# broadinstitute/colab-repeat-finder

Hardware: AMD Instinct MI355X
Metric: Gbp/s scanned (motif 1-50) (higher is better)
Workload: dtype u32 bit planes (2-bit bases)

## Files before the change

colab-repeat-finder_amd/csrc/plan.cpp:

```cpp
#include <algorithm>
#include <cstdio>
#include <cstdlib>
#include <cstring>
#include <string>
#include <vector>

#include "prf_plan.h"

using namespace prf_layout;
static constexpr int MAX_WAVES = PRF_VMAX_WAVES;

bool prf_vertical_plan(u32 kmin, u32 kmax, u32 min_repeats, u32 min_span, prf_vplan *plan) {
    if (kmin < 1 || kmax < kmin || kmax > PRF_VMAX_K || min_repeats < 2) return false;
    struct Item {
        prf_vtask t;
        u32 cost;
    };
    std::vector<Item> items;
    u32 reach = 0;
    u32 covered_to = 0;
    const bool derive_k1 = prf_plan_derives_k1(kmin, kmax, min_repeats, min_span);
    for (u32 k = kmin; k <= kmax; k++) {
        const long long M = prf_plan_min_matches(k, min_repeats, min_span);
        if (M < SMALL_M) {
            Item it;
            it.t.k0 = (unsigned short)k;
            it.t.kind = (unsigned char)M;
            it.t.valid = 1;
            it.t.stride = 1;
            it.t.pad = 0;
            it.cost = M <= 8 ? 660u : (M <= 10 ? 520u : 400u);
            if (derive_k1 && k == 1) {
                it.t.pad = PRF_TASK_DERIVED;
                it.cost = 0;
            }
            if (derive_k1 && k == 2) it.t.pad = PRF_TASK_RAISES_K1;
            items.push_back(it);
            reach = std::max<u32>(reach, 4 * (((u32)T + (u32)M - 1 + k + 3) / 4) - 1);
        } else if (k >= covered_to) {
            const u32 k0 = k & ~3u;
            u32 valid = 0;
            long long mmin[2] = {1ll << 40, 1ll << 40};
            for (u32 kk = 0; kk < 8; kk++) {
                const u32 kx = k0 + kk;
                const long long Mx = prf_plan_min_matches(kx, min_repeats, min_span);
                if (kx >= kmin && kx <= kmax && Mx >= SMALL_M) {
                    valid |= 1u << kk;
                    mmin[kk >> 2] = std::min(mmin[kk >> 2], Mx);
                }
            }
            auto stride_of = [](long long m) { return m >= 39 ? 4u : (m >= 23 ? 2u : 1u); };
            const bool both = (valid & 0x0Fu) && (valid & 0xF0u);
            if (both && stride_of(mmin[0]) != stride_of(mmin[1])) valid &= 0x0Fu;
            const bool half = (valid & 0xF0u) == 0;
            const u32 stride = stride_of(half ? mmin[0] : std::min(mmin[0], mmin[1]));
            Item it;
            it.t.k0 = (unsigned short)k0;
            it.t.kind = 0;
            it.t.valid = (unsigned char)valid;
            it.t.stride = (unsigned char)stride;
            it.t.pad = 0;
            const u32 n_sizes = (u32)__builtin_popcount(valid);
            it.cost = stride == 1 ? 155u + 125u * n_sizes : (stride == 2 ? 105u + 90u * n_sizes : 140u + 40u * n_sizes);
            items.push_back(it);
            reach = std::max<u32>(reach, 24 + k0 + (half ? 11 : 15));
            covered_to = k0 + (half ? 4 : 8);
        }
    }
    if (items.size() > PRF_VMAX_TASKS) return false;
    std::vector<Item> sorted;
    for (const Item &it : items)
        if (!(it.t.pad & PRF_TASK_DERIVED)) sorted.push_back(it);
    const u32 nw = std::max<u32>(1, std::min<u32>(PRF_VMAX_WAVES, (u32)sorted.size()));
    std::vector<std::vector<Item>> bins(nw);
    std::vector<u32> load(nw, 0);
    std::stable_sort(sorted.begin(), sorted.end(), [](const Item &a, const Item &b) { return a.cost > b.cost; });
    constexpr u32 TICKET_COST = 30;
    bool ticket_dealt = nw < (u32)PRF_VMAX_WAVES;
    plan->ticket_wave = nw < (u32)PRF_VMAX_WAVES ? nw : 0;
    for (const Item &it : sorted) {
        if (!ticket_dealt && it.cost <= TICKET_COST) {
            plan->ticket_wave = (u32)(std::min_element(load.begin(), load.end()) - load.begin());
            load[plan->ticket_wave] += TICKET_COST;
            ticket_dealt = true;
        }
        const u32 w = (u32)(std::min_element(load.begin(), load.end()) - load.begin());
        bins[w].push_back(it);
        load[w] += it.cost;
    }
    if (!ticket_dealt) {
        plan->ticket_wave = (u32)(std::min_element(load.begin(), load.end()) - load.begin());
        load[plan->ticket_wave] += TICKET_COST;
    }
    for (int round = 0; round < 64; round++) {
        const u32 hi = (u32)(std::max_element(load.begin(), load.end()) - load.begin());
        bool moved = false;
        for (u32 o = 0; o < nw && !moved; o++) {
            if (o == hi) continue;
            for (size_t i = 0; i < bins[hi].size() && !moved; i++) {
                const u32 ci = bins[hi][i].cost;
                if (std::max(load[hi] - ci, load[o] + ci) < load[hi]) {
                    bins[o].push_back(bins[hi][i]);
                    bins[hi].erase(bins[hi].begin() + (long)i);
                    load[hi] -= ci;
                    load[o] += ci;
                    moved = true;
                    break;
                }
                for (size_t j = 0; j < bins[o].size(); j++) {
                    const u32 cj = bins[o][j].cost;
                    if (cj < ci && std::max(load[hi] - ci + cj, load[o] + ci - cj) < load[hi]) {
                        std::swap(bins[hi][i], bins[o][j]);
                        load[hi] = load[hi] - ci + cj;
                        load[o] = load[o] + ci - cj;
                        moved = true;
                        break;
                    }
                }
            }
        }
        if (!moved) break;
    }
    auto rank_of = [](const Item &it) { return it.t.kind != 0 ? 1 : (it.t.stride < 4 ? 0 : 2); };
    for (auto &bin : bins)
        if (derive_k1) std::stable_sort(bin.begin(), bin.end(), [&](const Item &a, const Item &b) {
            if (rank_of(a) != rank_of(b)) return rank_of(a) < rank_of(b);
            return a.t.kind == 0 && a.t.k0 < b.t.k0;
        });
    for (const Item &it : items)
        if (it.t.pad & PRF_TASK_DERIVED)
            for (auto &bin : bins)
                for (size_t i = 0; i < bin.size(); i++)
                    if (bin[i].t.pad & PRF_TASK_RAISES_K1) {
                        bin.insert(bin.begin() + (long)i + 1, it);
                        break;
                    }
    {
#ifdef PRF_DIAG
        static const u32 prio_cfg = getenv("PRF_PRIO") ? (u32)strtoul(getenv("PRF_PRIO"), nullptr, 0) : 0xA02u;
#else
        const u32 prio_cfg = 0xA02u;
#endif
        plan->prio = prio_cfg;
        const u32 busiest = *std::max_element(load.begin(), load.end());
        plan->slack_waves = 0;
        for (u32 w = 0; w < (u32)PRF_VMAX_WAVES; w++)
            if (w >= nw || 10u * load[w] < 9u * busiest) plan->slack_waves |= 1u << w;
    }
    plan->n_waves = nw;
    plan->n_tasks = 0;
    plan->n_group_k = 0;
    plan->n_exact = 0;
    u32 k_exact0 = ~0u, k_exact1 = 0, n_exact_items = 0;
    for (const Item &it : items)
        if (it.t.kind) {
            k_exact0 = std::min<u32>(k_exact0, it.t.k0);
            k_exact1 = std::max<u32>(k_exact1, it.t.k0);
            n_exact_items++;
        }
    if (n_exact_items && k_exact1 - k_exact0 + 1 != n_exact_items) return false;
    plan->k_exact0 = n_exact_items ? k_exact0 : 0;
    for (u32 w = 0; w < nw; w++) {
        plan->wave_begin[w] = plan->n_tasks;
        for (const Item &it : bins[w]) {
            prf_vtask t = it.t;
            t.item0 = 0;
            if (t.kind == 0) {
                t.item0 = (unsigned short)plan->n_group_k;
                plan->n_group_k += (u32)__builtin_popcount((unsigned)t.valid);
            } else {
                plan->n_exact++;
                t.item0 = (unsigned short)(t.k0 - k_exact0);
            }
            plan->tasks[plan->n_tasks++] = t;
        }
    }
    for (u32 w = nw; w <= PRF_VMAX_WAVES; w++) plan->wave_begin[w] = plan->n_tasks;
    const u32 need_nc = 64 + reach / T;
    plan->nc = need_nc <= 72 ? 72 : 80;
    plan->cof_words = (kmax + 1 + 3) & ~3u;
    plan->lds_bytes = (u32)(SMEM_HDR + (size_t)2 * RG * plan->nc * 16 + (size_t)REC_CAP * sizeof(u64) +
                            (size_t)2 * ROW_CAP_LDS * sizeof(u32) + (size_t)SLOW_CAP * 16 + (size_t)FLAG_CAP * 2 +
                            (size_t)plan->n_group_k * sizeof(u32) + (size_t)plan->cof_words * sizeof(u32));
    plan->per_cu = 0;
    return need_nc <= 80;
}


int prf_plan_json(u32 kmin, u32 kmax, u32 min_repeats, u32 min_span, char *buf, u64 buf_len) {
    std::string out;
    prf_vplan plan;
    if (!prf_vertical_plan(kmin, kmax, min_repeats, min_span, &plan)) {
        out = "{\"path\": \"generic\"}";
    } else {
        char tmp[160];
        snprintf(tmp, sizeof tmp, "{\"path\": \"fused\", \"waves\": %u, \"nc\": %u, \"lds_bytes\": %u, \"tasks\": [", plan.n_waves,
                 plan.nc, plan.lds_bytes);
        out = tmp;
        bool first = true;
        for (u32 w = 0; w < plan.n_waves; w++)
            for (u32 ti = plan.wave_begin[w]; ti < plan.wave_begin[w + 1]; ti++) {
                const prf_vtask &t = plan.tasks[ti];
                snprintf(tmp, sizeof tmp, "%s{\"wave\": %u, \"kind\": %u, \"k0\": %u, \"valid\": %u, \"stride\": %u, \"derive\": %u}",
                         first ? "" : ", ", w, (unsigned)t.kind, (unsigned)t.k0, (unsigned)t.valid, (unsigned)t.stride, (unsigned)(t.pad & 3u));
                out += tmp;
                first = false;
            }
        out += "]}";
    }
    if (out.size() + 1 > buf_len) return -1;
    memcpy(buf, out.c_str(), out.size() + 1);
    return (int)out.size();
}
```

colab-repeat-finder_amd/csrc/scan_vertical.hip:

```cpp
#include <algorithm>
#include <cstdio>
#include <cstdlib>
#include <utility>
#include <vector>

#include "prf_host.h"
#include "prf_static_for.h"
#include "scan_vertical.h"
#include "verify_impl.h"

namespace {

#include "vscan_common.h"
#include "vscan_verify.h"
#include "vscan_tasks.h"

__device__ __forceinline__ void set_prio(u32 p) {
#ifdef PRF_NO_PRIO
    return;
#endif
    if (p == 0u) __builtin_amdgcn_s_setprio(0);
    else if (p == 1u) __builtin_amdgcn_s_setprio(1);
    else if (p == 2u) __builtin_amdgcn_s_setprio(2);
    else __builtin_amdgcn_s_setprio(3);
// ... 41 lines not shown
        if (ut < n_extra) {
            const u32 pw = (u32)__builtin_amdgcn_readfirstlane((int)(ut / (u32)(RG * extra)));
            const u32 erg = (ut / (u32)extra) % (u32)RG, el = ut % (u32)extra;
            const u32 i0 = (erg * 64u + el) * 16u, i1 = i0 + (u32)(RG * 64) * 16u;
            if (pw == 0) {
                ev = ld16(ph, i0);
                en = ld16(ph, i1);
            } else {
                ev = ld16(pL, i0);
                en = ld16(pL, i1);
            }
        }
    }
    __device__ __forceinline__ void clear() {
        const prf_u32x4 z = {0, 0, 0, 0};
        ev = en = z;
        entry = 0;
    }
    __device__ __forceinline__ void store(prf_lds_u4 *vimg, int tid) const {
        const u32 sx = (u32)tid;
        if (sx < n_extra) {
            const u32 p = sx / (u32)(RG * extra), erg = (sx / (u32)extra) % (u32)RG, el = sx % (u32)extra;
            vimg[p * RG * NC + erg * (u32)NC + 64u + el] = (ev >> 1) | (en << 31);
        }
    }
};

__device__ __forceinline__ u32 vscan_skip(const prf_vscan_args &g) {
#ifdef PRF_DIAG
    return g.skip;
#else
    (void)g;
    return 0u;
#endif
}

template <int NC>
__global__ __launch_bounds__(NTH, 6) void prf_vscan_kernel(prf_vscan_args g) {
    constexpr u32 R1_OFF = (u32)SMEM_HDR, R1_BYTES = (u32)(2 * RG * NC * 16);
    constexpr u32 RECS_OFF = R1_OFF + R1_BYTES, KEYS_OFF = RECS_OFF + (u32)REC_CAP * 8u, SLOW_OFF = KEYS_OFF + 2u * (u32)ROW_CAP_LDS * 4u,
                  HOTW_OFF = SLOW_OFF + (u32)SLOW_CAP * 16u, BITEMS_OFF = HOTW_OFF + (u32)FLAG_CAP * 2u;
    static_assert(SLOW_CAP * 16 >= 256, "the all-N stream masks lie in the deferred candidates' list");
    static_assert(2 * LW * 8 <= (int)R1_BYTES, "the window of the linear planes must fit the image's region");
    static_assert((2 * LW / 2 + 63) / 64 <= 5 * MAX_WAVES, "window pieces per wave");
    static_assert(LEAD_OFF == R1_OFF + 2u * (u32)LW * 8u && LEAD_OFF + 2u * LEAD_CAP * 4u <= R1_OFF + R1_BYTES, "the record waves' stream lists lie in R1 behind the window");
    prf_lds_u4 *vimg = (prf_lds_u4 *)(prf_smem + R1_OFF);
    prf_lds_u64 *recs = (prf_lds_u64 *)(prf_smem + RECS_OFF);
    prf_lds_u32 *keys = (prf_lds_u32 *)(prf_smem + KEYS_OFF);
    prf_lds_u32 *nostart = (prf_lds_u32 *)(prf_smem + SLOW_OFF);
    prf_lds_u32 *hotw = (prf_lds_u32 *)(prf_smem + HOTW_OFF);
    prf_lds_u32 *bitems = (prf_lds_u32 *)(prf_smem + BITEMS_OFF);

    const int tid0 = (int)threadIdx.x;
    const int wave = __builtin_amdgcn_readfirstlane(tid0 >> 6);
    auto entry_of = [&](u32 sl) -> u32 { return g.flat_base != ~0u ? g.flat_base + sl : g.launch_list[sl]; };

    set_prio(g.plan.prio & 3u);
    NextRegs<NC> sr;
    sr.load(g, entry_of(blockIdx.x), tid0, wave, R1_OFF);
    for (u32 v = (u32)tid0; v < 8u * g.plan.n_tasks; v += (u32)NTH) {
        const prf_vtask task = g.plan.tasks[v >> 3];
        const u32 kk = v & 7u;
        if (task.kind == 0 && ((task.valid >> kk) & 1u))
            bitems[(u32)task.item0 + (u32)__builtin_popcount((u32)task.valid & ((1u << kk) - 1u))] = ((u32)task.k0 + kk) | ((u32)task.stride << 16);
    }
    {
        prf_lds_u32 *cof_lds = bitems + g.plan.n_group_k;
        for (int i = tid0; i < (int)g.plan.cof_words; i += NTH) cof_lds[i] = prf_cof_table.v[i];
    }
    if (tid0 == 0) {
        TileCtx *tcw = reinterpret_cast<TileCtx *>(prf_smem);
        tcw->H = g.H; tcw->L = g.L; tcw->X = g.X;
        tcw->E = g.E;
        tcw->slab_cap = g.slab_cap;
        tcw->min_repeats = g.min_repeats;
        tcw->min_span = g.min_span;
        tcw->lin_off = R1_OFF;
        tcw->keys_off = KEYS_OFF;
        tcw->slow_off = SLOW_OFF;
        tcw->k_exact0 = g.plan.k_exact0;
        tcw->cof_off = BITEMS_OFF + 4u * g.plan.n_group_k;
    }

    const u32 xcd = blockIdx.x & 7u;
    const u32 first_ticket = (gridDim.x - xcd + 7u) >> 3;
    u64 *ticket_word = g.counters + (PRF_CNT_SHARD0 + xcd * PRF_CNT_SHARD_STRIDE + PRF_SH_TILE_TICKET);
    prf_lds_u32 *next_words = (prf_lds_u32 *)(prf_smem + HDR_NEXT);
    u32 slot_next = 0;
    u32 parity = 0;
    prf_lds_u32 *wg_stats = (prf_lds_u32 *)(prf_smem + HDR_STATS);
    if (tid0 == 0) wg_stats[0] = wg_stats[1] = 0;
    for (u32 slot = blockIdx.x; slot < g.n_launch; slot = slot_next, parity ^= 1u) {
    int wave_s = wave;
    asm volatile("" : "+s"(wave_s));
    u32 ones = ~0u;
    asm volatile("" : "+s"(ones));
    int tid = wave_s * 64 + (int)__builtin_amdgcn_mbcnt_hi(ones, __builtin_amdgcn_mbcnt_lo(ones, 0u));
    asm volatile("" : "+v"(tid));
    const int lane = tid & 63;
    const u32 entry = sr.entry;
    const bool hasx = (entry & PRF_LAUNCH_MIXED) != 0;
    const u64 tile = entry & ~PRF_LAUNCH_MIXED;
    prf_lds_u32 *cnt = smem_cnt(parity);

    PRF_STAMP(0);
#ifdef PRF_STAMPS
    if (g.dbg && lane == 0) g.dbg[((u64)slot * MAX_WAVES + wave) * PRF_STAMP_SLOTS + 12] = __builtin_amdgcn_s_memrealtime();
#endif
    set_prio(g.plan.prio & 3u);
    {
        sr.store(vimg, tid);
        if (hasx && tid < 64) {
            const u32 *px = reinterpret_cast<const u32 *>(g.X + tile * PRF_TILE_WORDS);
            u32 m = 0;
#pragma unroll 1
            for (u32 b0 = 0; b0 < 32u; b0 += 8u) {
                u32 v[8];
                static_for<0, 8>([&](auto bc) { v[decltype(bc)::value] = *(prf_glb_cu32 *)(px + ((b0 + (u32)decltype(bc)::value) * 64u + (u32)tid)); });
                static_for<0, 8>([&](auto bc) { m |= (v[decltype(bc)::value] == ~0u ? 1u : 0u) << (b0 + (u32)decltype(bc)::value); });
            }
            nostart[tid] = m;
        }
        if (tid < (int)CNT_N) cnt[tid] = 0;
        if (tid == 0) {
            TileCtx *tcw = reinterpret_cast<TileCtx *>(prf_smem);
            tcw->w0 = tile * PRF_TILE_WORDS - LIN_PRE;
            tcw->xz_lo = hasx ? 0 : tile * PRF_TILE;
            tcw->xz_hi = hasx ? 0 : (tile + 2) * PRF_TILE;
            tcw->slab = (prf_glb_u64 *)(g.slabs + (u64)slot * g.slab_cap);
            tcw->tile_base = tile * PRF_TILE;
            tcw->has_lin = 0u;
            tcw->cnt_off = (u32)HDR_CNT + 4u * CNT_N * parity;
        }
    }
    PRF_STAMP(1);
    __syncthreads();
    PRF_STAMP(2);

    set_prio(((g.plan.slack_waves >> wave) & 1u) ? (g.plan.prio >> 4) & 3u : (g.plan.prio >> 2) & 3u);
    Emit em;
    em.recs = recs;
    em.cnt = cnt;
    em.lane = lane;
#ifdef PRF_STAMPS
    u64 *task_dbg = g.dbg ? g.dbg + ((u64)slot * MAX_WAVES + wave) * PRF_STAMP_SLOTS : nullptr;
#else
    u64 *task_dbg = nullptr;
#endif
    {
        u32 allow = hasx ? ~nostart[lane] : ~0u;
        if (vscan_skip(g) & 1u) allow = 0u;
        run_tasks<NC>((prf_lds_cu4 *)vimg, hotw, nostart, g.plan, wave, lane, hasx, allow, em, task_dbg);
    }
    constexpr u32 WIN_UNITS = (u32)LW;
    constexpr u32 WIN_PIECES = (WIN_UNITS + 63u) / 64u;
    static_assert(WIN_PIECES == 17, "the window's pieces are dealt 9 + 8 to the first two waves to arrive");
    prf_u32x4 wv[9];
    u32 order = 0;
    {
        if (lane == 0) order = atomicAdd((u32 *)(cnt + CNT_ROWS0), 1u);
        order = (u32)__builtin_amdgcn_readfirstlane((int)order);
        const long long w0 = (long long)(tile * PRF_TILE_WORDS) - LIN_PRE;
        const u64 *wh = g.H + w0, *wl = g.L + w0;
        const prf_u32x4 z = {0, 0, 0, 0};
        static_for<0, 9>([&](auto ic) { wv[decltype(ic)::value] = z; });
        if (order < 2u) {
            const u32 first = order * 9u, n = order ? 8u : 9u;
            static_for<0, 9>([&](auto ic) {
                constexpr u32 i = (u32)decltype(ic)::value;
                if (i < n) {
                    const u32 u = (first + i) * 64u + (u32)lane;
                    const u64 *src = u < (u32)LW / 2u ? wh + 2u * u : wl + 2u * (u - (u32)LW / 2u);
                    if (u < WIN_UNITS) wv[i] = *reinterpret_cast<const prf_u32x4 *>(src);
                }
            });
        }
    }
    u64 ticket = 0;
    const bool ticket_thread = order == 0u && lane == 0;
    if (ticket_thread) ticket = atomicAdd(ticket_word, 1ull);
    PRF_STAMP(3);
    __syncthreads();
    {
        if (order < 2u) {
            const u32 first = order * 9u, n = order ? 8u : 9u;
            static_for<0, 9>([&](auto ic) {
                constexpr u32 i = (u32)decltype(ic)::value;
                if (i < n) {
                    const u32 u = (first + i) * 64u + (u32)lane;
                    if (u < WIN_UNITS) *(prf_lds_u4 *)(prf_smem + R1_OFF + 16u * u) = wv[i];
                }
            });
        }
        const prf_u32x4 n0 = *(prf_lds_cu4 *)(cnt + CNT_ROWS);
        for (u32 i = (u32)tid; i < (u32)ROW_CAP_LDS; i += (u32)NTH) {
            const u32 q = i / (u32)QCAP, j = i - q * (u32)QCAP;
            const u32 n0q = q == 0u ? n0.x : (q == 1u ? n0.y : (q == 2u ? n0.z : n0.w));
            if (j >= n0q) keys[i] = quarter_pad(q);
        }
        if (tid == 0) {
            reinterpret_cast<TileCtx *>(prf_smem)->has_lin = 1u;
            cnt[CNT_ROWS0] = n0.x;
            cnt[CNT_ROWS0 + 1u] = n0.y;
            cnt[CNT_ROWS0 + 2u] = n0.z;
            cnt[CNT_ROWS0 + 3u] = n0.w;
            cnt[CNT_OVF0] = cnt[CNT_OVF];
            cnt[CNT_LONG0] = cnt[CNT_LONG];
        }
    }
    u32 slot_pre = 0, entry_pre = entry;
    if (ticket_thread) {
        slot_pre = (first_ticket + (u32)ticket) * 8u + xcd;
        if (slot_pre < g.n_launch) entry_pre = entry_of(slot_pre);
    }
    __syncthreads();
    PRF_STAMP(4);

    set_prio(wave < MAX_WAVES / 2 ? (g.plan.prio >> 6) & 3u : (g.plan.prio >> 8) & 3u);
    const u32 *xw = hasx ? reinterpret_cast<const u32 *>(g.X + ((long long)(tile * PRF_TILE_WORDS) - LIN_PRE)) : nullptr;
    typedef const unsigned short __attribute__((address_space(3))) prf_lds_cu16;
    u32 n_recs = cnt[CNT_RECS], n_flags = cnt[CNT_FLAGS];
    {
        if (tid == 0) {
            const u32 early = cnt[CNT_EARLY];
            wg_stats[0] += n_flags + n_recs + early;
            wg_stats[1] += early;
        }
        n_recs = n_recs < (u32)REC_CAP ? n_recs : (u32)REC_CAP;
        n_flags = n_flags < (u32)FLAG_CAP ? n_flags : (u32)FLAG_CAP;
#ifdef PRF_STAMPS
        if (g.dbg && tid == 0) g.dbg[((u64)slot * MAX_WAVES + 0) * PRF_STAMP_SLOTS + 11] = (u64)n_flags | ((u64)n_recs << 32);
#endif
        if (vscan_skip(g) & 2u) n_flags = 0;
        if (vscan_skip(g) & 4u) n_recs = 0;
        verify_all((prf_lds_cu64 *)recs, n_recs, (prf_lds_cu32 *)bitems, (vscan_skip(g) & 8u) ? 0u : g.plan.n_group_k, (prf_lds_cu16 *)hotw, n_flags, xw, (u32)tid, task_dbg);
    }
    set_prio((g.plan.prio >> 10) & 3u);
    if (ticket_thread) {
        next_words[0] = slot_pre;
        next_words[1] = entry_pre;
    }
    PRF_STAMP(5);
    __syncthreads();
    {
        const u32 n_slow = (u32)__builtin_amdgcn_readfirstlane((int)cnt[CNT_SLOW]);
        if (n_slow) {
            if (n_slow <= (u32)SLOW_CAP) {
                if ((u32)tid < n_slow) {
                    prf_lds_u64 *slow = (prf_lds_u64 *)(prf_smem + SLOW_OFF);
                    slow_item(slow[2u * (u32)tid], slow[2u * (u32)tid + 1u]);
                }
            } else {
                if (tid == 0) {
                    for (u32 q = 0; q < 4u; q++) cnt[CNT_ROWS + q] = cnt[CNT_ROWS0 + q];
                    cnt[CNT_OVF] = cnt[CNT_OVF0];
                    cnt[CNT_LONG] = cnt[CNT_LONG0];
                }
                __syncthreads();
                verify_general((prf_lds_cu64 *)recs, n_recs, (prf_lds_cu32 *)bitems, g.plan.n_group_k, (prf_lds_cu16 *)hotw, n_flags, (u32)tid);
            }
            __syncthreads();
        }
    }
    PRF_STAMP(6);
    const u64 nw = *(prf_lds_u64 *)next_words;
    slot_next = (u32)__builtin_amdgcn_readfirstlane((int)(u32)nw);
    const u32 entry_next = (u32)(nw >> 32);
    u32 nq0, nq1, nq2, nq3;
    {
        const prf_u32x4 c = *(prf_lds_cu4 *)(cnt + CNT_ROWS);
        const bool none = (vscan_skip(g) & 16u) != 0;
        nq0 = none ? 0u : (u32)__builtin_amdgcn_readfirstlane((int)c.x);
        nq1 = none ? 0u : (u32)__builtin_amdgcn_readfirstlane((int)c.y);
        nq2 = none ? 0u : (u32)__builtin_amdgcn_readfirstlane((int)c.z);
        nq3 = none ? 0u : (u32)__builtin_amdgcn_readfirstlane((int)c.w);
    }
    const u32 n_rows = nq0 + nq1 + nq2 + nq3;
    const bool dense = nq0 > (u32)QCAP || nq1 > (u32)QCAP || nq2 > (u32)QCAP || nq3 > (u32)QCAP;
    const u32 n_long = (u32)__builtin_amdgcn_readfirstlane((int)cnt[CNT_LONG]);
    u64 *slab = g.slabs + (u64)slot * g.slab_cap;
    const u32 n_store = n_rows < g.slab_cap ? n_rows : g.slab_cap;
    bool unsorted = false;
    if (tid == 0) {
        g.slab_count[slot] = n_rows;
        if (n_store && !(vscan_skip(g) & 32u)) atomicAdd(&g.block_sum[slot >> g.gather_shift], n_store);
    }

    if (dense) {
        constexpr u32 R1_ROWS = R1_BYTES / 8u;
        const u32 m0 = nq0 < (u32)QCAP ? nq0 : (u32)QCAP, m1 = nq1 < (u32)QCAP ? nq1 : (u32)QCAP, m2 = nq2 < (u32)QCAP ? nq2 : (u32)QCAP,
                  m3 = nq3 < (u32)QCAP ? nq3 : (u32)QCAP;
        const u32 n_ovf = n_rows - (m0 + m1 + m2 + m3);
        const u32 s1 = nq0, s2 = nq0 + nq1, s3 = s2 + nq2;
        auto pick = [](u32 q, u32 a0, u32 a1, u32 a2, u32 a3) -> u32 { return q == 0u ? a0 : (q == 1u ? a1 : (q == 2u ? a2 : a3)); };
        if (n_rows <= g.slab_cap && n_rows <= R1_ROWS) {
            prf_lds_u32 *k2 = (prf_lds_u32 *)(prf_smem + R1_OFF), *v2 = k2 + R1_ROWS;
            prf_lds_u32 *fill = cnt + CNT_ROWS0;
            if (tid < 4) fill[tid] = pick((u32)tid, m0, m1, m2, m3);
            for (u32 i = (u32)tid; i < (u32)ROW_CAP_LDS; i += (u32)NTH) {
                const u32 q = i / (u32)QCAP, j = i - q * (u32)QCAP;
                if (j < pick(q, m0, m1, m2, m3)) {
                    const u32 at = pick(q, 0u, s1, s2, s3) + j;
                    k2[at] = keys[i];
                    v2[at] = keys[ROW_CAP_LDS + i];
                }
            }
            __syncthreads();
            for (u32 i = (u32)tid; i < n_ovf; i += (u32)NTH) {
                const u64 r = slab[i];
                const u32 q = (u32)r >> 30;
                const u32 at = pick(q, 0u, s1, s2, s3) + atomicAdd((u32 *)(fill + q), 1u);
                k2[at] = (u32)r;
                v2[at] = (u32)(r >> 32);
            }
            for (u32 i = n_rows + (u32)tid; i < ((n_rows + 3u) & ~3u); i += (u32)NTH) k2[i] = 0xFFFFFFFFu;
            __syncthreads();
            typedef __attribute__((address_space(3))) const prf_u32x4 prf_lds_ckey4;
            prf_lds_ckey4 *k4 = (prf_lds_ckey4 *)k2;
            for (u32 r = (u32)tid; r < n_rows; r += (u32)NTH) {
                const u32 mine = k2[r], kv = v2[r];
                const u32 q = mine >> 30;
                const u32 lo = pick(q, 0u, s1, s2, s3), hi = lo + pick(q, nq0, nq1, nq2, nq3);
                const u32 u_lo = lo >> 2, u_hi = (hi + 3u) >> 2;
                u32 rank = 4u * u_lo;
#pragma unroll 4
                for (u32 u = u_lo; u < u_hi; u++) {
                    const prf_u32x4 v = k4[u];
                    rank += (v.x < mine ? 1u : 0u) + (v.y < mine ? 1u : 0u) + (v.z < mine ? 1u : 0u) + (v.w < mine ? 1u : 0u);
                }
                slab[rank] = (u64)mine | ((u64)kv << 32);
            }
            __syncthreads();
        } else {
            for (u32 i = (u32)tid; i < (u32)ROW_CAP_LDS; i += (u32)NTH) {
                const u32 q = i / (u32)QCAP, j = i - q * (u32)QCAP;
                const u32 at = n_ovf + pick(q, 0u, m0, m0 + m1, m0 + m1 + m2) + j;
                if (j < pick(q, m0, m1, m2, m3) && at < g.slab_cap) slab[at] = (u64)keys[i] | ((u64)keys[ROW_CAP_LDS + i] << 32);
            }
            unsorted = true;
        }
    }

    if (slot_next < g.n_launch) sr.load(g, entry_next, tid, wave, R1_OFF);
    else sr.clear();

    PRF_RANK_DECL();
    {
        const u32 nq = wave_s == 0 ? nq0 : (wave_s == 1 ? nq1 : (wave_s == 2 ? nq2 : nq3));
        const u32 below = wave_s == 0 ? 0u : (wave_s == 1 ? nq0 : (wave_s == 2 ? nq0 + nq1 : nq0 + nq1 + nq2));
        if (nq && !dense) {
            const u32 lg = nq > 32u ? 0u : (nq > 16u ? 1u : 2u);
            const u32 P = 1u << lg, part = (u32)lane & (P - 1u);
            const u32 units = (nq + 3u) >> 2;
            prf_lds_u32 *sub = keys + (u32)wave_s * (u32)QCAP;
            typedef __attribute__((address_space(3))) const prf_u32x4 prf_lds_ckey4;
            prf_lds_ckey4 *k4 = (prf_lds_ckey4 *)sub + part;
            for (u32 row0 = 0; row0 < nq; row0 += 64u >> lg) {
                const u32 row = row0 + ((u32)lane >> lg);
                const u32 r = row < nq ? row : 0u;
                PRF_RANK_T0();
                const u32 mine = sub[r];
                const u32 kv = sub[ROW_CAP_LDS + r];
                u32 rank = 0;
                auto batch = [&](u32 u0, auto nc) {
                    constexpr u32 N = (u32)decltype(nc)::value;
                    prf_u32x4 v[N];
                    static_for<0, (int)N>([&](auto jc) { v[decltype(jc)::value] = k4[u0 + (u32)decltype(jc)::value * P]; });
                    if constexpr (N == 4u) asm volatile("" : "+v"(v[0]), "+v"(v[1]), "+v"(v[2]), "+v"(v[3]));
                    else asm volatile("" : "+v"(v[0]), "+v"(v[1]));
                    u32 bits = 0;
                    static_for<0, (int)N>([&](auto jc) {
                        constexpr u32 j = (u32)decltype(jc)::value;
                        bits = __builtin_amdgcn_alignbit(bits, v[j].x - mine, 31);
                        bits = __builtin_amdgcn_alignbit(bits, v[j].y - mine, 31);
                        bits = __builtin_amdgcn_alignbit(bits, v[j].z - mine, 31);
                        bits = __builtin_amdgcn_alignbit(bits, v[j].w - mine, 31);
                    });
                    rank += (u32)__builtin_popcount(bits);
                };
                for (u32 u0 = 0; u0 < units; u0 += 4u * P) {
                    if (units - u0 > 2u * P) batch(u0, std::integral_constant<u32, 4>{});
                    else batch(u0, std::integral_constant<u32, 2>{});
                }
                if (P >= 2u) rank += (u32)__builtin_amdgcn_update_dpp(0, (int)rank, 0xB1, 0xF, 0xF, true);
// ... 72 lines not shown
```

colab-repeat-finder_amd/csrc/vscan_tasks.h:

```cpp

struct Emit {
    prf_lds_u64 *recs;
    prf_lds_u32 *cnt;
    int lane;
#ifdef PRF_STAMPS
    u64 t_push_g = 0, t_push_f = 0;
#endif

    static constexpr u32 DENSE_FLAGS = 4;
    __device__ __forceinline__ void push_flags(u32 word, u32 e, u32 k, prf_lds_u32 *flag_words) {
        typedef __attribute__((address_space(3))) unsigned short prf_lds_u16;
        prf_lds_u16 *list = (prf_lds_u16 *)flag_words;
        const u32 pc = (u32)__builtin_popcount(word);
        if (__builtin_amdgcn_ballot_w64(pc > DENSE_FLAGS) != 0) {
            push_flags_levels(word, e, k, list);
            return;
        }
        if (word == 0) return;
        u32 at = atomicAdd((u32 *)(cnt + CNT_FLAGS), pc);
        const u32 tag = (u32)lane | (e << 11);
        if (at + pc <= (u32)FLAG_CAP) {
            prf_lds_u16 *p = list + at;
            do {
                *p++ = (unsigned short)(tag | ((u32)__builtin_ctz(word) << 6));
// ... 267 lines not shown
                    const u32 win = window_or<M, t>(mm, o3);
                    if constexpr (!ECHO) {
                        if constexpr (t >= 0) hot = bitop3<(TA | (~TB & TC)) & 0xFF>(hot, win, prev);
                        if constexpr (t == 0) {
                            if (relax) hot |= ~win;
                        }
                    } else if constexpr (t >= 0) {
                        if constexpr (t == 0 || t % SEG == 1) seg = ~win & prev;
                        else seg = bitop3<(TA | (~TB & TC)) & 0xFF>(seg, win, prev);
                        if constexpr (t == 0) {
                            if (relax) seg |= ~win;
                        }
                        if constexpr (t % SEG == 0 || t == T - 1) {
                            hot = bitop3<(TA | (TB & TC)) & 0xFF>(hot, seg, prim[(t + SEG - 1) / SEG]);
                            if constexpr (K == 2) hot1 = bitop3<(TA | (TB & ~TC)) & 0xFF>(hot1, seg, prim[(t + SEG - 1) / SEG]);
                        }
                    }
                    prev = win;
                }
            }
        });
    });
    return (u64)hot | ((u64)hot1 << 32);
}

template <int K, int M, int NC>
__device__ __attribute__((noinline)) u32 coarse_stream(prf_lds_cu4 *vimg, int lane, bool relax) {
    constexpr int PS = RG * NC;
    constexpr int G = M >= 11 ? 4 : 2, C = (M + 1) / G - 1;
    constexpr int NJ = T / G + 1;
    constexpr int NGRP = NJ + C;
    constexpr int NR = T + G * C;
    constexpr int NG = (NR + K + 3) / 4;
    static_assert(C >= 2 && 4 * NG <= 2 * T, "a coarse task reads its own lane and the next one");
    int lane_o = lane;
    asm volatile("" : "+v"(lane_o));
    prf_lds_cu4 *lane_base = vimg + lane_o;
    u32 q0[4], q1[4];
    {
        const int pl = (lane + 63) & 63;
        prf_lds_cu4 *pp = vimg + pl + (RG - 1) * NC;
        prf_u32x4 v0 = pp[0], v1 = pp[PS];
        if (lane == 0) {
            v0 <<= 1;
            v1 <<= 1;
        }
        q0[0] = v0.x; q0[1] = v0.y; q0[2] = v0.z; q0[3] = v0.w;
        q1[0] = v1.x; q1[1] = v1.y; q1[2] = v1.z; q1[3] = v1.w;
    }
    u32 r0[4 * NG], r1[4 * NG];
    u32 grp[NGRP];
    u32 hot = 0;
    auto load_slot = [&](auto gc) {
        constexpr int g = decltype(gc)::value;
        if constexpr (g < NG) {
            prf_lds_cu4 *ps = slot_of<NC>(lane_base, g);
            const prf_u32x4 v0 = ps[0], v1 = ps[PS];
            r0[4 * g] = v0.x; r0[4 * g + 1] = v0.y; r0[4 * g + 2] = v0.z; r0[4 * g + 3] = v0.w;
            r1[4 * g] = v1.x; r1[4 * g + 1] = v1.y; r1[4 * g + 2] = v1.z; r1[4 * g + 3] = v1.w;
        }
    };
    auto h = [&](auto rc) -> u32 { constexpr int r = decltype(rc)::value; if constexpr (r < 0) return q0[r + 4]; else return r0[r]; };
    auto l = [&](auto rc) -> u32 { constexpr int r = decltype(rc)::value; if constexpr (r < 0) return q1[r + 4]; else return r1[r]; };
    load_slot(std::integral_constant<int, 0>{});
    static_for<0, NG>([&](auto gc) {
        constexpr int g = decltype(gc)::value;
        load_slot(std::integral_constant<int, g + 1>{});
        __builtin_amdgcn_sched_barrier(0);
        static_for<0, 4>([&](auto jc) {
            constexpr int i = 4 * g + decltype(jc)::value - K;
            if constexpr (i >= -1 && i < NR && (i + 1) % G == 0) {
                constexpr int j = (i + 1) / G - 1, first = G * j;
                u32 t = h(std::integral_constant<int, first>{}) ^ h(std::integral_constant<int, first + K>{});
                t = or_xor(t, l(std::integral_constant<int, first>{}), l(std::integral_constant<int, first + K>{}));
                static_for<1, G>([&](auto ic) {
                    constexpr int r = first + decltype(ic)::value;
                    t = or_xor(t, h(std::integral_constant<int, r>{}), h(std::integral_constant<int, r + K>{}));
                    t = or_xor(t, l(std::integral_constant<int, r>{}), l(std::integral_constant<int, r + K>{}));
                });
                if constexpr (j == -1) {
                    if (lane == 0) t |= 1u;
                }
                grp[j + 1] = t;
                constexpr int w = j - C + 1;
                if constexpr (w >= 0 && w < NJ) {
                    u32 win;
                    if constexpr (C == 2) win = grp[w + 1] | grp[w + 2];
                    else if constexpr (C == 3) win = or3(grp[w + 1], grp[w + 2], grp[w + 3]);
                    else if constexpr (C == 4) win = or3(grp[w + 1], grp[w + 2], grp[w + 3]) | grp[w + 4];
                    else win = or3(or3(grp[w + 1], grp[w + 2], grp[w + 3]), grp[w + 4], grp[w + 5]);
                    static_assert(C <= 5, "window of at most five groups");
                    hot = bitop3<(TA | (~TB & TC)) & 0xFF>(hot, win, grp[w]);
                    if constexpr (w == 0) {
                        if (relax) hot |= ~win;
                    }
                }
            }
        });
    });
    return hot;
}

constexpr int exact_variants() { return (SMALL_M - 1) * SMALL_M / 2; }
constexpr int exact_variant_of(int K, int M) { return (K - 1) * (2 * SMALL_M - K) / 2 + (M - K); }
constexpr int exact_variant_k(int v) {
    int K = 1;
    while (exact_variant_of(K + 1, K + 1) <= v) K++;
    return K;
}
template <int LO, int HI, int NC>
__device__ __forceinline__ u64 exact_dispatch(prf_lds_cu4 *vimg, int lane, bool relax, u32 v) {
    if constexpr (LO == HI) {
        constexpr int K = exact_variant_k(LO), M = K + (LO - exact_variant_of(K, K));
        static_assert(M >= K && M < SMALL_M && exact_variant_of(K, M) == LO, "variant numbering");
        if constexpr (M >= 9) return coarse_stream<K, M, NC>(vimg, lane, relax);
        else return exact_stream<K, M, NC>(vimg, lane, relax);
    } else {
        constexpr int MID = (LO + HI) / 2;
        if (v <= (u32)MID) return exact_dispatch<LO, MID, NC>(vimg, lane, relax, v);
        return exact_dispatch<MID + 1, HI, NC>(vimg, lane, relax, v);
    }
}

template <int NC>
__device__ __forceinline__ u64 exact_any(prf_lds_cu4 *vimg, int lane, bool relax, u32 k, u32 M) {
    const u32 v = (k - 1u) * (2u * (u32)SMALL_M - k) / 2u + (M - k);
    return exact_dispatch<0, exact_variants() - 1, NC>(vimg, lane, relax, v);
}

template <int NC>
__device__ __forceinline__ void run_tasks(prf_lds_cu4 *vimg, prf_lds_u32 *hotw, prf_lds_u32 *k1w, const prf_vplan &plan, int wave, int lane, bool relax,
                                          u32 allow, Emit &em, u64 *dbg) {
    const u32 t_end = plan.wave_begin[wave + 1];
    {
        u32 a = (u32)(__UINTPTR_TYPE__)vimg;
        asm volatile("" : "+s"(a));
        vimg = (prf_lds_cu4 *)(__UINTPTR_TYPE__)a;
    }
#ifdef PRF_STAMPS
    u64 t_call = 0;
#endif
    for (u32 ti = plan.wave_begin[wave]; ti < t_end; ti++) {
        static_assert(sizeof(prf_vtask) == 8 && alignof(prf_vtask) == 4, "a task is read as two dwords");
        const u32 *tw = reinterpret_cast<const u32 *>(&plan.tasks[ti]);
        const u32 tw0 = (u32)__builtin_amdgcn_readfirstlane((int)tw[0]), tw1 = (u32)__builtin_amdgcn_readfirstlane((int)tw[1]);
        prf_vtask task;
        task.k0 = (unsigned short)(tw0 & 0xFFFFu);
        task.kind = (unsigned char)((tw0 >> 16) & 0xFFu);
        task.valid = (unsigned char)(tw0 >> 24);
        task.stride = (unsigned char)(tw1 & 0xFFu);
        task.pad = (unsigned char)((tw1 >> 8) & 0xFFu);
        task.item0 = (unsigned short)(tw1 >> 16);
#ifdef PRF_STAMPS
        if (dbg && lane == 0 && ti - plan.wave_begin[wave] < 8u) dbg[8 + (ti - plan.wave_begin[wave])] = __builtin_amdgcn_s_memtime();
#endif
        if (task.kind == 0) {
            const bool half = (task.valid & 0xF0u) == 0;
            if (task.stride == 1 && !relax) {
                if (half) group_task<NC, true, true>(vimg, lane, task.k0, task.valid, 1u, allow, em);
                else group_task<NC, true, false>(vimg, lane, task.k0, task.valid, 1u, allow, em);
            } else {
                if (half) group_task<NC, false, true>(vimg, lane, task.k0, task.valid, task.stride, allow, em);
                else group_task<NC, false, false>(vimg, lane, task.k0, task.valid, task.stride, allow, em);
            }
        } else {
            u32 word;
#ifdef PRF_STAMPS
            const u64 tc0 = __builtin_amdgcn_s_memtime();
#endif
            if ((task.pad & PRF_TASK_DERIVED) && !relax) {
                word = k1w[lane];
            } else {
                const u64 words = exact_any<NC>(vimg, lane, relax, task.k0, task.kind);
                word = (u32)words & allow;
                if ((task.pad & PRF_TASK_RAISES_K1) && !relax) k1w[lane] = (u32)(words >> 32) & allow;
            }
#ifdef PRF_STAMPS
            asm volatile("" ::"v"(word));
            const u64 tc1 = __builtin_amdgcn_s_memtime();
            t_call += tc1 - tc0;
#endif
            em.push_flags(word, task.item0, task.k0, hotw);
#ifdef PRF_STAMPS
            em.t_push_f += __builtin_amdgcn_s_memtime() - tc1;
#endif
        }
    }
#ifdef PRF_STAMPS
    if (dbg && lane == 0) dbg[15] = (t_call & 0x3FFFFFull) | ((em.t_push_f & 0x1FFFFFull) << 22) | ((em.t_push_g & 0x1FFFFFull) << 43);
#endif
}
```

Baseline: 6665.

## Rebalance wave task deal with measured prices, local search and exhaustive search

Replaces the per-task cost model with new task prices and folds the k=1 derived handover cost into the task that raises it. Greedy dealing is now followed by move/swap local search and, for small task counts, an exhaustive branch-and-bound over wave assignments. The ticket wave is chosen from the final loads, and wave priority is raised after the task phase. The window registers are left uninitialised instead of being zeroed. The plan is cached per parameter set so repeated host calls skip the search. The aim is to shorten the busiest wave's critical path, at the risk that the price model does not match the real kernel.

```diff
diff --git a/colab-repeat-finder_amd/csrc/plan.cpp b/colab-repeat-finder_amd/csrc/plan.cpp
--- a/colab-repeat-finder_amd/csrc/plan.cpp
+++ b/colab-repeat-finder_amd/csrc/plan.cpp
@@ -10,7 +10,77 @@
 using namespace prf_layout;
 static constexpr int MAX_WAVES = PRF_VMAX_WAVES;
 
-bool prf_vertical_plan(u32 kmin, u32 kmax, u32 min_repeats, u32 min_span, prf_vplan *plan) {
+namespace {
+constexpr u32 FIRST_TASK = 300;
+constexpr u32 K1_HANDOVER = 1660;
+
+u32 task_price(const prf_vtask &t) {
+    if (t.kind != 0) {
+        if (t.pad & PRF_TASK_DERIVED) return K1_HANDOVER;
+        const u32 k = t.k0, M = t.kind;
+        if (M <= 8) {
+            if (k == 2 && M == 7) return 4000;
+            if (k == 3 && M == 6) return 4040;
+            if (k == 4 && M == 8) return 3960;
+            return 4000;
+        }
+        return M <= 10 ? 3630 : 3600;
+    }
+    const u32 n = (u32)__builtin_popcount((unsigned)t.valid);
+    if (t.stride == 1) return 3050 + 400 * n;
+    if (t.stride == 2) return 3550 + 200 * n;
+    return 2900 + 100 * n;
+}
+
+#ifdef PRF_DIAG
+const u32 WINDOW_W = getenv("PRF_PLAN_W") ? (u32)strtoul(getenv("PRF_PLAN_W"), nullptr, 0) : 0u;
+#else
+constexpr u32 WINDOW_W = 0;
+#endif
+
+constexpr u32 PRIO_HANDOVER = 3, PRIO_FLAGS = 2;
+
+struct DealKey {
+    u32 obj, a4, a34;
+    bool operator<(const DealKey &o) const { return obj != o.obj ? obj < o.obj : (a4 != o.a4 ? a4 < o.a4 : a34 < o.a34); }
+};
+DealKey deal_key(const u32 (&load)[PRF_VMAX_WAVES]) {
+    u32 a[PRF_VMAX_WAVES];
+    std::copy(load, load + PRF_VMAX_WAVES, a);
+    std::sort(a, a + PRF_VMAX_WAVES);
+    return DealKey{std::max(a[PRF_VMAX_WAVES - 1], a[1] + WINDOW_W), a[PRF_VMAX_WAVES - 1], a[PRF_VMAX_WAVES - 1] + a[PRF_VMAX_WAVES - 2]};
+}
+
+struct DealSearch {
+    const std::vector<u32> &cost;
+    std::vector<u32> where, best_where;
+    u32 load[PRF_VMAX_WAVES] = {};
+    DealKey best;
+    long nodes = 0;
+    static constexpr long MAX_NODES = 400000;
+    void go(size_t i) {
+        if (++nodes > MAX_NODES) return;
+        const DealKey here = deal_key(load);
+        if (!(here < best)) return;
+        if (i == cost.size()) {
+            best = here;
+            best_where = where;
+            return;
+        }
+        for (u32 w = 0; w < (u32)PRF_VMAX_WAVES; w++) {
+            bool seen = false;
+            for (u32 v = 0; v < w; v++) seen = seen || load[v] == load[w];
+            if (seen) continue;
+            load[w] += cost[i];
+            where[i] = w;
+            go(i + 1);
+            load[w] -= cost[i];
+        }
+    }
+};
+}
+
+static bool build_plan(u32 kmin, u32 kmax, u32 min_repeats, u32 min_span, prf_vplan *plan) {
     if (kmin < 1 || kmax < kmin || kmax > PRF_VMAX_K || min_repeats < 2) return false;
     struct Item {
         prf_vtask t;
@@ -29,12 +99,9 @@
             it.t.valid = 1;
             it.t.stride = 1;
             it.t.pad = 0;
-            it.cost = M <= 8 ? 660u : (M <= 10 ? 520u : 400u);
-            if (derive_k1 && k == 1) {
-                it.t.pad = PRF_TASK_DERIVED;
-                it.cost = 0;
-            }
+            if (derive_k1 && k == 1) it.t.pad = PRF_TASK_DERIVED;
             if (derive_k1 && k == 2) it.t.pad = PRF_TASK_RAISES_K1;
+            it.cost = task_price(it.t);
             items.push_back(it);
             reach = std::max<u32>(reach, 4 * (((u32)T + (u32)M - 1 + k + 3) / 4) - 1);
         } else if (k >= covered_to) {
@@ -60,8 +127,7 @@
             it.t.valid = (unsigned char)valid;
             it.t.stride = (unsigned char)stride;
             it.t.pad = 0;
-            const u32 n_sizes = (u32)__builtin_popcount(valid);
-            it.cost = stride == 1 ? 155u + 125u * n_sizes : (stride == 2 ? 105u + 90u * n_sizes : 140u + 40u * n_sizes);
+            it.cost = task_price(it.t);
             items.push_back(it);
             reach = std::max<u32>(reach, 24 + k0 + (half ? 11 : 15));
             covered_to = k0 + (half ? 4 : 8);
@@ -69,58 +135,77 @@
     }
     if (items.size() > PRF_VMAX_TASKS) return false;
     std::vector<Item> sorted;
+    u32 handover = 0;
     for (const Item &it : items)
-        if (!(it.t.pad & PRF_TASK_DERIVED)) sorted.push_back(it);
-    const u32 nw = std::max<u32>(1, std::min<u32>(PRF_VMAX_WAVES, (u32)sorted.size()));
+        if (it.t.pad & PRF_TASK_DERIVED) handover = it.cost;
+        else sorted.push_back(it);
+    for (Item &it : sorted)
+        if (it.t.pad & PRF_TASK_RAISES_K1) it.cost += handover;
+    std::stable_sort(sorted.begin(), sorted.end(), [](const Item &a, const Item &b) { return a.cost > b.cost; });
+    const size_t n_dealt = sorted.size();
+    std::vector<u32> cost(n_dealt), where(n_dealt, 0);
+    u32 load[PRF_VMAX_WAVES] = {};
+    for (size_t i = 0; i < n_dealt; i++) {
+        cost[i] = sorted[i].cost;
+        where[i] = (u32)(std::min_element(load, load + PRF_VMAX_WAVES) - load);
+        load[where[i]] += cost[i];
+    }
+    for (bool better = true; better;) {
+        better = false;
+        DealKey cur = deal_key(load);
+        for (size_t i = 0; i < n_dealt && !better; i++) {
+            for (u32 w = 0; w < (u32)PRF_VMAX_WAVES && !better; w++) {
+                if (w == where[i]) continue;
+                u32 l2[PRF_VMAX_WAVES];
+                std::copy(load, load + PRF_VMAX_WAVES, l2);
+                l2[where[i]] -= cost[i];
+                l2[w] += cost[i];
+                if (deal_key(l2) < cur) {
+                    std::copy(l2, l2 + PRF_VMAX_WAVES, load);
+                    where[i] = w;
+                    better = true;
+                }
+            }
+            for (size_t j = i + 1; j < n_dealt && !better; j++) {
+                if (where[i] == where[j] || cost[i] == cost[j]) continue;
+                u32 l2[PRF_VMAX_WAVES];
+                std::copy(load, load + PRF_VMAX_WAVES, l2);
+                l2[where[i]] = l2[where[i]] - cost[i] + cost[j];
+                l2[where[j]] = l2[where[j]] - cost[j] + cost[i];
+                if (deal_key(l2) < cur) {
+                    std::copy(l2, l2 + PRF_VMAX_WAVES, load);
+                    std::swap(where[i], where[j]);
+                    better = true;
+                }
+            }
+        }
+    }
+    constexpr size_t EXHAUSTIVE_TASKS = 16;
+    if (n_dealt <= EXHAUSTIVE_TASKS) {
+        DealSearch ds{cost, std::vector<u32>(n_dealt, 0), where};
+        ds.best = deal_key(load);
+        ds.go(0);
+        where = ds.best_where;
+    }
+    u32 n_used = 0;
+    {
+        u32 name[PRF_VMAX_WAVES];
+        std::fill(name, name + PRF_VMAX_WAVES, ~0u);
+        for (size_t i = 0; i < n_dealt; i++)
+            if (name[where[i]] == ~0u) name[where[i]] = n_used++;
+        for (size_t i = 0; i < n_dealt; i++) where[i] = name[where[i]];
+    }
+    const u32 nw = std::max<u32>(1, n_used);
     std::vector<std::vector<Item>> bins(nw);
-    std::vector<u32> load(nw, 0);
-    std::stable_sort(sorted.begin(), sorted.end(), [](const Item &a, const Item &b) { return a.cost > b.cost; });
-    constexpr u32 TICKET_COST = 30;
-    bool ticket_dealt = nw < (u32)PRF_VMAX_WAVES;
-    plan->ticket_wave = nw < (u32)PRF_VMAX_WAVES ? nw : 0;
-    for (const Item &it : sorted) {
-        if (!ticket_dealt && it.cost <= TICKET_COST) {
-            plan->ticket_wave = (u32)(std::min_element(load.begin(), load.end()) - load.begin());
-            load[plan->ticket_wave] += TICKET_COST;
-            ticket_dealt = true;
-        }
-        const u32 w = (u32)(std::min_element(load.begin(), load.end()) - load.begin());
-        bins[w].push_back(it);
-        load[w] += it.cost;
-    }
-    if (!ticket_dealt) {
-        plan->ticket_wave = (u32)(std::min_element(load.begin(), load.end()) - load.begin());
-        load[plan->ticket_wave] += TICKET_COST;
-    }
-    for (int round = 0; round < 64; round++) {
-        const u32 hi = (u32)(std::max_element(load.begin(), load.end()) - load.begin());
-        bool moved = false;
-        for (u32 o = 0; o < nw && !moved; o++) {
-            if (o == hi) continue;
-            for (size_t i = 0; i < bins[hi].size() && !moved; i++) {
-                const u32 ci = bins[hi][i].cost;
-                if (std::max(load[hi] - ci, load[o] + ci) < load[hi]) {
-                    bins[o].push_back(bins[hi][i]);
-                    bins[hi].erase(bins[hi].begin() + (long)i);
-                    load[hi] -= ci;
-                    load[o] += ci;
-                    moved = true;
-                    break;
-                }
-                for (size_t j = 0; j < bins[o].size(); j++) {
-                    const u32 cj = bins[o][j].cost;
-                    if (cj < ci && std::max(load[hi] - ci + cj, load[o] + ci - cj) < load[hi]) {
-                        std::swap(bins[hi][i], bins[o][j]);
-                        load[hi] = load[hi] - ci + cj;
-                        load[o] = load[o] + ci - cj;
-                        moved = true;
-                        break;
-                    }
-                }
-            }
-        }
-        if (!moved) break;
-    }
+    std::fill(load, load + PRF_VMAX_WAVES, 0u);
+    for (size_t i = 0; i < n_dealt; i++) {
+        Item it = sorted[i];
+        load[where[i]] += it.cost;
+        if (it.t.pad & PRF_TASK_RAISES_K1) it.cost -= handover;
+        bins[where[i]].push_back(it);
+    }
+    for (u32 w = 0; w < nw; w++) load[w] += FIRST_TASK;
+    plan->ticket_wave = (u32)(std::min_element(load, load + PRF_VMAX_WAVES) - load);
     auto rank_of = [](const Item &it) { return it.t.kind != 0 ? 1 : (it.t.stride < 4 ? 0 : 2); };
     for (auto &bin : bins)
         if (derive_k1) std::stable_sort(bin.begin(), bin.end(), [&](const Item &a, const Item &b) {
@@ -136,13 +221,14 @@
                         break;
                     }
     {
+        constexpr u32 PRIO_DEFAULT = 0x0A02u | (PRIO_HANDOVER << 12) | (PRIO_FLAGS << 6);
 #ifdef PRF_DIAG
-        static const u32 prio_cfg = getenv("PRF_PRIO") ? (u32)strtoul(getenv("PRF_PRIO"), nullptr, 0) : 0xA02u;
+        static const u32 prio_cfg = getenv("PRF_PRIO") ? (u32)strtoul(getenv("PRF_PRIO"), nullptr, 0) : PRIO_DEFAULT;
 #else
-        const u32 prio_cfg = 0xA02u;
+        const u32 prio_cfg = PRIO_DEFAULT;
 #endif
         plan->prio = prio_cfg;
-        const u32 busiest = *std::max_element(load.begin(), load.end());
+        const u32 busiest = *std::max_element(load, load + PRF_VMAX_WAVES);
         plan->slack_waves = 0;
         for (u32 w = 0; w < (u32)PRF_VMAX_WAVES; w++)
             if (w >= nw || 10u * load[w] < 9u * busiest) plan->slack_waves |= 1u << w;
@@ -186,6 +272,23 @@
     return need_nc <= 80;
 }
 
+bool prf_vertical_plan(u32 kmin, u32 kmax, u32 min_repeats, u32 min_span, prf_vplan *plan) {
+    struct Last {
+        u32 key[4];
+        bool have, ok;
+        prf_vplan plan;
+    };
+    thread_local Last last = {};
+    if (!(last.have && last.key[0] == kmin && last.key[1] == kmax && last.key[2] == min_repeats && last.key[3] == min_span)) {
+        last.have = false;
+        last.plan = prf_vplan{};
+        last.ok = build_plan(kmin, kmax, min_repeats, min_span, &last.plan);
+        last.key[0] = kmin; last.key[1] = kmax; last.key[2] = min_repeats; last.key[3] = min_span;
+        last.have = true;
+    }
+    *plan = last.plan;
+    return last.ok;
+}
 
 int prf_plan_json(u32 kmin, u32 kmax, u32 min_repeats, u32 min_span, char *buf, u64 buf_len) {
     std::string out;
@@ -193,16 +296,17 @@
     if (!prf_vertical_plan(kmin, kmax, min_repeats, min_span, &plan)) {
         out = "{\"path\": \"generic\"}";
     } else {
-        char tmp[160];
-        snprintf(tmp, sizeof tmp, "{\"path\": \"fused\", \"waves\": %u, \"nc\": %u, \"lds_bytes\": %u, \"tasks\": [", plan.n_waves,
-                 plan.nc, plan.lds_bytes);
+        char tmp[240];
+        snprintf(tmp, sizeof tmp, "{\"path\": \"fused\", \"waves\": %u, \"nc\": %u, \"lds_bytes\": %u, \"window\": %u, \"first_task\": %u, \"tasks\": [",
+                 plan.n_waves, plan.nc, plan.lds_bytes, (unsigned)WINDOW_W, (unsigned)FIRST_TASK);
         out = tmp;
         bool first = true;
         for (u32 w = 0; w < plan.n_waves; w++)
             for (u32 ti = plan.wave_begin[w]; ti < plan.wave_begin[w + 1]; ti++) {
                 const prf_vtask &t = plan.tasks[ti];
-                snprintf(tmp, sizeof tmp, "%s{\"wave\": %u, \"kind\": %u, \"k0\": %u, \"valid\": %u, \"stride\": %u, \"derive\": %u}",
-                         first ? "" : ", ", w, (unsigned)t.kind, (unsigned)t.k0, (unsigned)t.valid, (unsigned)t.stride, (unsigned)(t.pad & 3u));
+                snprintf(tmp, sizeof tmp, "%s{\"wave\": %u, \"kind\": %u, \"k0\": %u, \"valid\": %u, \"stride\": %u, \"derive\": %u, \"price\": %u}",
+                         first ? "" : ", ", w, (unsigned)t.kind, (unsigned)t.k0, (unsigned)t.valid, (unsigned)t.stride, (unsigned)(t.pad & 3u),
+                         (unsigned)task_price(t));
                 out += tmp;
                 first = false;
             }
diff --git a/colab-repeat-finder_amd/csrc/scan_vertical.hip b/colab-repeat-finder_amd/csrc/scan_vertical.hip
--- a/colab-repeat-finder_amd/csrc/scan_vertical.hip
+++ b/colab-repeat-finder_amd/csrc/scan_vertical.hip
@@ -217,6 +217,8 @@
         if (vscan_skip(g) & 1u) allow = 0u;
         run_tasks<NC>((prf_lds_cu4 *)vimg, hotw, nostart, g.plan, wave, lane, hasx, allow, em, task_dbg);
     }
+    PRF_STAMP(17);
+    set_prio((g.plan.prio >> 12) & 3u);
     constexpr u32 WIN_UNITS = (u32)LW;
     constexpr u32 WIN_PIECES = (WIN_UNITS + 63u) / 64u;
     static_assert(WIN_PIECES == 17, "the window's pieces are dealt 9 + 8 to the first two waves to arrive");
@@ -225,10 +227,12 @@
     {
         if (lane == 0) order = atomicAdd((u32 *)(cnt + CNT_ROWS0), 1u);
         order = (u32)__builtin_amdgcn_readfirstlane((int)order);
+#ifdef PRF_STAMPS
+        if (g.dbg && lane == 0) g.dbg[((u64)slot * MAX_WAVES + wave) * PRF_STAMP_SLOTS + 18] = order;
+#endif
         const long long w0 = (long long)(tile * PRF_TILE_WORDS) - LIN_PRE;
         const u64 *wh = g.H + w0, *wl = g.L + w0;
-        const prf_u32x4 z = {0, 0, 0, 0};
-        static_for<0, 9>([&](auto ic) { wv[decltype(ic)::value] = z; });
+        asm("" : "=v"(wv[0]), "=v"(wv[1]), "=v"(wv[2]), "=v"(wv[3]), "=v"(wv[4]), "=v"(wv[5]), "=v"(wv[6]), "=v"(wv[7]), "=v"(wv[8]));
         if (order < 2u) {
             const u32 first = order * 9u, n = order ? 8u : 9u;
             static_for<0, 9>([&](auto ic) {
@@ -244,8 +248,19 @@
     u64 ticket = 0;
     const bool ticket_thread = order == 0u && lane == 0;
     if (ticket_thread) ticket = atomicAdd(ticket_word, 1ull);
-    PRF_STAMP(3);
+#ifdef PRF_STAMPS
+    {
+        const u64 t3 = __builtin_amdgcn_s_memtime();
+        if (order < 2u) asm volatile("s_waitcnt vmcnt(0)" ::: "memory");
+        const u64 t20 = __builtin_amdgcn_s_memtime();
+        if (g.dbg && lane == 0) {
+            g.dbg[((u64)slot * MAX_WAVES + wave) * PRF_STAMP_SLOTS + 3] = t3;
+            g.dbg[((u64)slot * MAX_WAVES + wave) * PRF_STAMP_SLOTS + 20] = t20;
+        }
+    }
+#endif
     __syncthreads();
+    PRF_STAMP(19);
     {
         if (order < 2u) {
             const u32 first = order * 9u, n = order ? 8u : 9u;
@@ -257,6 +272,7 @@
                 }
             });
         }
+        PRF_STAMP(21);
         const prf_u32x4 n0 = *(prf_lds_cu4 *)(cnt + CNT_ROWS);
         for (u32 i = (u32)tid; i < (u32)ROW_CAP_LDS; i += (u32)NTH) {
             const u32 q = i / (u32)QCAP, j = i - q * (u32)QCAP;
@@ -272,6 +288,7 @@
             cnt[CNT_OVF0] = cnt[CNT_OVF];
             cnt[CNT_LONG0] = cnt[CNT_LONG];
         }
+        PRF_STAMP(22);
     }
     u32 slot_pre = 0, entry_pre = entry;
     if (ticket_thread) {
@@ -294,7 +311,7 @@
         n_recs = n_recs < (u32)REC_CAP ? n_recs : (u32)REC_CAP;
         n_flags = n_flags < (u32)FLAG_CAP ? n_flags : (u32)FLAG_CAP;
 #ifdef PRF_STAMPS
-        if (g.dbg && tid == 0) g.dbg[((u64)slot * MAX_WAVES + 0) * PRF_STAMP_SLOTS + 11] = (u64)n_flags | ((u64)n_recs << 32);
+        if (g.dbg && tid == 0) g.dbg[((u64)slot * MAX_WAVES + 0) * PRF_STAMP_SLOTS + 23] = (u64)n_flags | ((u64)n_recs << 32);
 #endif
         if (vscan_skip(g) & 2u) n_flags = 0;
         if (vscan_skip(g) & 4u) n_recs = 0;
diff --git a/colab-repeat-finder_amd/csrc/vscan_tasks.h b/colab-repeat-finder_amd/csrc/vscan_tasks.h
--- a/colab-repeat-finder_amd/csrc/vscan_tasks.h
+++ b/colab-repeat-finder_amd/csrc/vscan_tasks.h
@@ -443,7 +443,7 @@
         task.pad = (unsigned char)((tw1 >> 8) & 0xFFu);
         task.item0 = (unsigned short)(tw1 >> 16);
 #ifdef PRF_STAMPS
-        if (dbg && lane == 0 && ti - plan.wave_begin[wave] < 8u) dbg[8 + (ti - plan.wave_begin[wave])] = __builtin_amdgcn_s_memtime();
+        if (dbg && lane == 0 && ti - plan.wave_begin[wave] < 4u) dbg[8 + (ti - plan.wave_begin[wave])] = __builtin_amdgcn_s_memtime();
 #endif
         if (task.kind == 0) {
             const bool half = (task.valid & 0xF0u) == 0;
```

Result: faster. 6748, median of 6 (+1.3%).
